# mutiann/few-shot-transformer-tts

Measured on AMD Instinct MI355X. Metric: padded mel-frames/sec, full training step (fwd+loss+bwd+allreduce+Adam), higher is better.
Workload: dtype bf16; 1 GPU; LJSpeech-shaped (BASELINE configs[1]) packed batch per GPU: B=14 S=114 T=582, default hparams (83.5M params), dropout on, single speaker/language; global_batch=14, seq_len=582, parallelism=dp1

## Files before the change

few-shot-transformer-tts_amd/csrc/engine.hip:

```cpp
#include <algorithm>
#include <cmath>
#include <cstdarg>
#include <cstdlib>
#include "engine.h"
#include "attention.h"
#include "enc_fused.h"
#include "drop_sites.h"

thread_local char g_b2s_err[512] = "";
int b2s_fail(const char* file, int line, const char* fmt, ...) {
    char msg[400];
    va_list ap; va_start(ap, fmt); vsnprintf(msg, sizeof(msg), fmt, ap); va_end(ap);
    const char* base = strrchr(file, '/');
    snprintf(g_b2s_err, sizeof(g_b2s_err), "%s:%d: %s", base ? base + 1 : file, line, msg);
    return 1;
}

int b2s_model::id(const std::string& n) const {
    auto it = index.find(n);
    return it == index.end() ? -1 : it->second;
}

namespace {

// ... 1457 lines not shown
            B2S_TRY(ro_cast(dt, memory, c->memT, Mk * D, st));
            if (c->kvcat)
                B2S_TRY(linear(m, st, c->memT, D, m->kv_cat, (int)Mk, cf.n_decoder_layer * 2 * D, D, c->kvcat, 0, cf.n_decoder_layer * 2 * D,
                               GemmEpilogue()));
            return 0;
        };
        if (!memory_ready) B2S_TRY(need_memory());
        if (c->ragged) {
            B2S_TRY(ro_set_rowoff(hoff.data(), B + 1, c->rowoff, st));
            B2S_TRY(ro_rows_gather(dt, targets, c->tgtT, roff, B, T, NM, st));
        } else B2S_TRY(ro_cast(dt, targets, c->tgtT, M * NM, st));
        GemmEpilogue e0; e0.bias = m->P("decoder.prenet.dense0.bias"); e0.relu = 1; e0.drop = make_drop(pd, seed, drop_op(DS_DEC_PRENET0, 0));
        B2S_TRY(linear(m, st, c->tgtT, NM, m->W("decoder.prenet.dense0.weight"), (int)Mr, HP, NM, c->a1, 0, HP, e0));
        GemmEpilogue e1; e1.bias = m->P("decoder.prenet.dense1.bias"); e1.relu = 1; e1.drop = make_drop(pd, seed, drop_op(DS_DEC_PRENET1, 0));
        B2S_TRY(linear(m, st, c->a1, HP, m->W("decoder.prenet.dense1.weight"), (int)Mr, HP, HP, c->a2, 0, HP, e1));
        B2S_TRY(linear(m, st, c->a2, HP, m->W("decoder.prenet.dense_final.weight"), (int)Mr, D, HP, sc.a3, 1, D, GemmEpilogue()));
        B2S_TRY(ro_shift_pe_fwd(sc.a3, target_lengths, m->pe_dec, m->P(p + "pe_scale"), xs[0], B, T, D,
                                make_drop(pt, seed, drop_op(DS_DEC_EMBED, 0)), st, roff, (int)Mr));
        const bool guided = cf.guided_attention_weight > 0.f;
        constexpr bool no_qskip = false;
        const int* qskip = (no_qskip || !padded_unobserved) ? nullptr : target_lengths;
        if (guided) {
            hipLaunchKernelGGL(k_ga_scale, dim3(1), dim3(64), 0, st, input_lengths, target_lengths, B, S, T,
                               cf.guided_attention_weight / (float)(cf.n_decoder_layer * H), c->ga_small);
            if (c->ragged) B2S_HIP(hipMemsetAsync(c->ga_rows, 0, (size_t)cf.n_decoder_layer * B * H * T * sizeof(float), st));
        }
        for (int l = 0; l < cf.n_decoder_layer; ++l) {
            AttnSave& s = c->self_attn[l]; AttnSave& x = c->cross_attn[l]; FfnSave& f = c->ffn[l];
            float* x0 = xs[3 * l]; float* x1 = xs[3 * l + 1]; float* x2 = xs[3 * l + 2]; float* x3 = xs[3 * l + 3];
            const std::string lna = p + "attn_layer_norms." + std::to_string(l);
            B2S_TRY(ro_layernorm_fwd(dt, x0, m->P(lna + ".weight"), m->P(lna + ".bias"), s.h, D, nullptr, 0, s.mean, s.rstd, (int)Mr, D,
                                     1e-6f, nullptr, 1, st));
            B2S_TRY(linear(m, st, s.h, D, m->W(nm(p, "self_attentions", l, "qkv_transform.weight")), (int)Mr, 3 * D, D, s.qkv, 0, 3 * D,
                           GemmEpilogue()));
            s.op_attn = drop_op(DS_DEC_SELF_ATTN, l); s.op_res = drop_op(DS_DEC_SELF_RES, l);
            const char* q = (const char*)s.qkv;
            B2S_TRY(attn_core_fwd(dt, st, q, 3 * D, q + (size_t)D * esz, 3 * D, q + (size_t)2 * D * esz, 3 * D, s.ctx, D, B, H, T, T, dh,
                                  2, nullptr, nullptr, 0, 0, make_drop(pt, seed, s.op_attn), sc.S, s.P, s.Pd, s.lse, nullptr, qskip, roff, roff));
            s.mask_mode = 2; s.qskip = qskip; s.qoff = s.koff = roff;
            GemmEpilogue ea; ea.drop = make_drop(pt, seed, s.op_res); ea.residual = x0; ea.ldr = D;
            B2S_TRY(linear(m, st, s.ctx, D, m->W(nm(p, "self_attentions", l, "output_transform.weight")), (int)Mr, D, D, x1, 1, D, ea));
            const std::string lnx = p + "encdec_layer_norms." + std::to_string(l);
            B2S_TRY(ro_layernorm_fwd(dt, x1, m->P(lnx + ".weight"), m->P(lnx + ".bias"), x.h, D, nullptr, 0, x.mean, x.rstd, (int)Mr, D,
                                     1e-6f, nullptr, 1, st));
            B2S_TRY(linear(m, st, x.h, D, m->W(nm(p, "encdec_attentions", l, "q_transform.weight")), (int)Mr, D, D, x.qkv, 0, D, GemmEpilogue()));
            B2S_TRY(need_memory());
            if (!c->kvcat)
                B2S_TRY(linear(m, st, c->memT, D, m->W(nm(p, "encdec_attentions", l, "kv_transform.weight")), (int)Mk, 2 * D, D, x.kv, 0, 2 * D,
                               GemmEpilogue()));
            x.op_attn = drop_op(DS_DEC_CROSS_ATTN, l); x.op_res = drop_op(DS_DEC_CROSS_RES, l);
            const char* kv = (const char*)x.kv;
            GuidedArgs ga;
            if (guided) {
                ga.rows = c->ga_rows + (long)l * B * H * T; ga.qlen = target_lengths;
                ga.inv2s2 = 1.f / (2.f * cf.guided_attention_sigma * cf.guided_attention_sigma);
            }
            B2S_TRY(attn_core_fwd(dt, st, x.qkv, D, kv, x.ldkv, kv + (size_t)D * esz, x.ldkv, x.ctx, D, B, H, T, S, dh, 1, input_lengths,
                                  nullptr, 0, 0, make_drop(pt, seed, x.op_attn), sc.S, x.P, x.Pd, x.lse, guided ? &ga : nullptr, qskip, roff, nullptr));
            x.mask_mode = 1; x.qskip = qskip; x.qoff = roff;
            GemmEpilogue ex; ex.drop = make_drop(pt, seed, x.op_res); ex.residual = x1; ex.ldr = D;
            B2S_TRY(linear(m, st, x.ctx, D, m->W(nm(p, "encdec_attentions", l, "output_transform.weight")), (int)Mr, D, D, x2, 1, D, ex));
            const std::string lnf = p + "ffn_layer_norms." + std::to_string(l);
            B2S_TRY(ro_layernorm_fwd(dt, x2, m->P(lnf + ".weight"), m->P(lnf + ".bias"), f.h, D, nullptr, 0, f.mean, f.rstd, (int)Mr, D,
                                     1e-6f, nullptr, 1, st));
            f.op_hid = drop_op(DS_DEC_FFN_HID, l); f.op_res = drop_op(DS_DEC_FFN_RES, l);
            GemmEpilogue f1; f1.relu = 1; f1.drop = make_drop(pt, seed, f.op_hid);
            B2S_TRY(linear(m, st, f.h, D, m->W(nm(p, "ffn_layers", l, "input_layer.weight")), (int)Mr, 4 * D, D, f.f, 0, 4 * D, f1));
            GemmEpilogue f2; f2.drop = make_drop(pt, seed, f.op_res); f2.residual = x2; f2.ldr = D;
            B2S_TRY(linear(m, st, f.f, 4 * D, m->W(nm(p, "ffn_layers", l, "output_layer.weight")), (int)Mr, D, 4 * D, x3, 1, D, f2));
        }
        B2S_TRY(need_memory());
        B2S_TRY(ro_layernorm_fwd(dt, c->x_final, m->P(p + "output_layer_norm.weight"), m->P(p + "output_layer_norm.bias"), c->outT, D,
                                 nullptr, 0, c->mean_f, c->rstd_f, (int)Mr, D, 1e-6f, c->ragged ? nullptr : target_lengths, T, st));
        GemmEpilogue em;
        if (!c->ragged) { em.row_len = target_lengths; em.rows_per_batch = T; }
        B2S_TRY(linear(m, st, c->outT, D, m->W("decoder.mel_net.weight"), (int)Mr, NM, D, c->ragged ? c->melc : mels_out, 1, NM, em));
        if (c->ragged)
            B2S_TRY(ro_heads_scatter(dt, c->outT, D, m->P("decoder.stop_net.weight"), m->P("decoder.stop_net.bias"), c->melc, mels_out, stop_out, roff, B, T, NM, D, st));
        else
            B2S_TRY(ro_rowdot_fwd(dt, c->outT, D, m->P("decoder.stop_net.weight"), m->P("decoder.stop_net.bias"), stop_out, (int)Mr, D, target_lengths, T, st));
        if (guided) hipLaunchKernelGGL(k_ga_reduce, dim3(1), dim3(1024), 0, st, c->ga_rows, (long)cf.n_decoder_layer * B * H * T, c->ga_small);
        B2S_LAUNCH_CHECK();
        return 0;
    };
    int rc = run();
    if (rc || !ctx_out) { delete c; if (ctx_out) *ctx_out = nullptr; return rc; }
    *ctx_out = c;
    return 0;
}

namespace {
__global__ void k_rowmask_copy(const float* in, float* out, const int* lens, int T, long n) {
    long i = (long)blockIdx.x * blockDim.x + threadIdx.x;
    if (i < n) { int b = (int)(i / T), t = (int)(i - (long)b * T); out[i] = t < lens[b] ? in[i] : 0.f; }
}
}

extern "C" int b2s_decoder_guided_loss(b2s_model* m, b2s_ctx* c, float* out, float* add_to, void* stream) {
    B2S_CHECK(m && c && c->kind == 2 && out, "bad decoder context");
    B2S_CHECK(c->ga_small, "guided_attention_weight is 0: this forward has no guided-attention term");
    hipLaunchKernelGGL(k_ga_fetch, dim3(1), dim3(1), 0, S_(stream), c->ga_small, out, add_to);
    B2S_LAUNCH_CHECK();
    return 0;
}
extern "C" int b2s_decoder_backward(b2s_model* m, b2s_ctx* c, const float* d_mels, const float* d_stop, const float* d_guided,
                                    int flags, float* d_memory_out, void* dmem_done, void* stream) {
    B2S_TRY(check_bound(m));
    const bool want_dmem = !(flags & B2S_DEC_BWD_NO_DMEMORY);
    B2S_CHECK(c && c->kind == 2 && d_mels && (d_memory_out || !want_dmem), "bad decoder context");
    const b2s_config& cf = m->cfg;
    hipStream_t st = S_(stream);
    const int B = c->B, S = c->S, T = c->T, D = cf.decoder_hidden, H = cf.n_attention_head, dh = D / H, dt = m->dtype, esz = m->esz;
    const int NM = cf.num_mels, HP = cf.prenet_hidden;
    const long Mp = (long)B * T, Mk = (long)B * S;
    const long M = c->ragged ? c->Mr : Mp;
    const int* roff = c->ragged ? c->rowoff : nullptr;
    const float pt = c->train ? cf.transformer_dropout_rate : 0.f, pd = c->train ? cf.decoder_dropout_rate : 0.f;
    Arena a; a.base = c->ws; a.cap = c->ws_bytes;
    b2s_ctx tmp; tmp.B = B; tmp.S = S; tmp.T = T; tmp.train = c->train;
    Scratch sc; std::vector<float*> xs;
    plan_decoder(m, tmp, a, sc, xs);
    const std::string p = "decoder.decoder.";
    const bool guided = c->ga_small != nullptr && d_guided != nullptr;
    if (guided) hipLaunchKernelGGL(k_ga_bscale, dim3(1), dim3(1), 0, st, c->ga_small, d_guided);
    if (c->ragged) B2S_TRY(ro_rows_gather(dt, d_mels, sc.dmelT, roff, B, T, NM, st, d_stop, sc.dstop_m, 1));
    else B2S_TRY(ro_cast(dt, d_mels, sc.dmelT, M * NM, st));
    B2S_TRY(linear_dw(m, st, sc.dmelT, NM, c->outT, D, (int)M, NM, D, m->G("decoder.mel_net.weight")));
    GemmEpilogue eo;
    if (!c->ragged) { eo.row_len = c->tgt_len; eo.rows_per_batch = T; }
    B2S_TRY(linear_dx(m, st, sc.dmelT, NM, m->W("decoder.mel_net.weight"), (int)M, D, NM, sc.doutT, 0, D, eo));
    if (d_stop) {
        if (!c->ragged) hipLaunchKernelGGL(k_rowmask_copy, dim3(cdiv(M, 256)), dim3(256), 0, st, d_stop, sc.dstop_m, c->tgt_len, T, M);
        B2S_TRY(grad_colsum(m, st, dt, c->outT, 0, D, sc.dstop_m, m->G("decoder.stop_net.weight"), 1, (int)M, D));
        B2S_TRY(grad_colsum(m, st, 0, sc.dstop_m, 1, 1, nullptr, m->G("decoder.stop_net.bias"), 1, (int)M, 1));
    }
    DropCfg nd;
    if (cf.n_decoder_layer > 0) nd = make_drop(pt, c->seed, c->ffn[cf.n_decoder_layer - 1].op_res);
    B2S_TRY(ln_bwd_exit(m, st, sc, sc.doutT, 0, D, c->x_final, p + "output_layer_norm", c->mean_f, c->rstd_f, 0, M, D, c->ragged ? nullptr : c->tgt_len, T,
                        cf.n_decoder_layer > 0 ? &nd : nullptr));
    B2S_TRY(end_stage(m, st, 1, false));
#ifdef B2S_LAB
    static const int tail_layers = getenv("B2S_LAB_DW_TAIL_LAYERS") ? atoi(getenv("B2S_LAB_DW_TAIL_LAYERS")) : 1;
    static const int tail_cap = getenv("B2S_LAB_DW_TAIL_CAP") ? atoi(getenv("B2S_LAB_DW_TAIL_CAP")) : 200;
#else
    constexpr int tail_layers = 1;
    constexpr int tail_cap = 200;
#endif
    m->dw_hold_from = -1; m->dw_tail_cap = 0;
    struct TailPolicyReset { b2s_model* m; ~TailPolicyReset() { m->dw_hold_from = -1; m->dw_tail_cap = 0; m->dw_flush_capped = false; } } tail_policy_reset{m};
    if ((flags & B2S_DEC_BWD_FLUSH_TAIL) && m->dw_group && tail_layers > 0 && tail_cap > 0 && dt == 1) {
        m->dw_hold_from = 2 + std::max(0, cf.n_decoder_layer - tail_layers);
        m->dw_tail_cap = tail_cap;
    }
    bool first_mem = true, dmem_finished = false;
    m->side_ev = nullptr;
    struct SideReset { b2s_model* m; ~SideReset() { m->side_ev = nullptr; } } side_reset{m};
    const bool side = m->side && m->side != st && sc.dkvcat && sc.dctx_x && dt == 1 && b2s_flash_supported(dh);
    if (side && m->side_evs.empty()) {
        m->side_evs.resize(16);
        for (auto& e : m->side_evs) B2S_HIP(hipEventCreateWithFlags(&e, hipEventDisableTiming));
    }
    auto finish_dmem = [&]() -> int {
        if (dmem_finished) return 0;
        dmem_finished = true;
        if (m->side_ev) { B2S_HIP(hipStreamWaitEvent(st, m->side_ev, 0)); m->side_ev = nullptr; }
        if (want_dmem && sc.dkvcat && cf.n_decoder_layer > 0) {
            const int Kc = cf.n_decoder_layer * 2 * D;
            GemmArgs g;
            g.A.p = sc.dkvcat; g.A.ld = Kc; g.A.R = (int)Mk; g.A.C = Kc;
            g.B.p = m->kv_cat; g.B.ld = D; g.B.R = Kc; g.B.C = D;
            g.M = (int)Mk; g.N = D; g.K = Kc; g.C = d_memory_out; g.c_fp32 = 1; g.ldc = D;
            if (m->dw_group) {
                B2S_HIP(hipMemsetAsync(d_memory_out, 0, (size_t)Mk * D * 4, st));
                g.epi.accumulate = 1; g.splitk = 4;
                m->set_ws(g, st);
            }
            B2S_TRY(b2s_gemm_launch(g, dt, false, true, st));
        } else if (first_mem && want_dmem) B2S_HIP(hipMemsetAsync(d_memory_out, 0, (size_t)Mk * D * 4, st));
        if (dmem_done) B2S_HIP(hipEventRecord((hipEvent_t)dmem_done, st));
        return 0;
    };
    for (int l = cf.n_decoder_layer - 1; l >= 0; --l) {
        const std::string lnf = p + "ffn_layer_norms." + std::to_string(l), lnx = p + "encdec_layer_norms." + std::to_string(l),
                          lna = p + "attn_layer_norms." + std::to_string(l);
        nd = make_drop(pt, c->seed, c->cross_attn[l].op_res);
        B2S_TRY(ffn_bwd(m, st, c->ffn[l], sc, M, D, pt, c->seed, nm(p, "ffn_layers", l, "input_layer.weight"),
                        nm(p, "ffn_layers", l, "output_layer.weight"), lnf, &nd));
        {
            const AttnSave& x = c->cross_attn[l];
            const std::string wq = nm(p, "encdec_attentions", l, "q_transform.weight"), wkv = nm(p, "encdec_attentions", l, "kv_transform.weight"),
                              wo = nm(p, "encdec_attentions", l, "output_transform.weight");
            DropCfg dres = make_drop(pt, c->seed, x.op_res), datt = make_drop(pt, c->seed, x.op_attn);
            const void* dy;
            B2S_TRY(take_dy(m, st, sc, M, D, dres, &dy));
            B2S_TRY(linear_dw(m, st, dy, D, x.ctx, D, (int)M, D, D, m->G(wo)));
            void* const dctx = side ? sc.dctx_x : sc.dctx;
            float* const dsum = side ? sc.dsum_x : sc.dP;
            if (side && m->side_ev) B2S_HIP(hipStreamWaitEvent(st, m->side_ev, 0));
            B2S_TRY(linear_dx(m, st, dy, D, m->W(wo), (int)M, D, D, dctx, 0, D, GemmEpilogue()));
            sc.dqkv = Scratch::rot(sc.r_dqkv, sc.i_dqkv);
            B2S_TRY(guard_write(m, sc.dqkv, st));
            int lddkv = 2 * D;
            if (sc.dkvcat) { sc.dkv = (char*)sc.dkvcat + (size_t)l * 2 * D * esz; lddkv = cf.n_decoder_layer * 2 * D; }
            else { sc.dkv = Scratch::rot(sc.r_dkv, sc.i_dkv); B2S_TRY(guard_write(m, sc.dkv, st)); }
            const char* kv = (const char*)x.kv; char* dkv = (char*)sc.dkv;
            GuidedArgs ga;
            if (guided) {
                ga.rows = c->ga_rows + (long)l * B * H * T; ga.qlen = c->tgt_len; ga.scale = c->ga_small + 2;
                ga.inv2s2 = 1.f / (2.f * cf.guided_attention_sigma * cf.guided_attention_sigma);
            }
            B2S_TRY(attn_core_bwd(dt, st, dctx, D, x.qkv, D, kv, x.ldkv, kv + (size_t)D * esz, x.ldkv, x.P, x.Pd, sc.dqkv, D, dkv, lddkv,
                                  dkv + (size_t)D * esz, lddkv, B, H, T, S, dh, datt, dsum, sc.dS, x.lse, x.ctx, x.mask_mode, c->in_len,
                                  guided ? &ga : nullptr, x.qskip, x.qoff, x.koff, side ? m->side : nullptr, side ? m->next_event() : nullptr));
            if (side) {
                hipEvent_t e = m->side_evs[m->side_next++ % m->side_evs.size()];
                B2S_HIP(hipEventRecord(e, m->side));
                m->side_ev = e;
            }
            B2S_TRY(linear_dw(m, st, sc.dqkv, D, x.h, D, (int)M, D, D, m->G(wq)));
            B2S_TRY(linear_dx(m, st, sc.dqkv, D, m->W(wq), (int)M, D, D, sc.dh, 0, D, GemmEpilogue()));
            B2S_TRY(linear_dw(m, st, sc.dkv, lddkv, c->memT, D, (int)Mk, 2 * D, D, m->G(wkv)));
            if (want_dmem && !sc.dkvcat) {
                GemmEpilogue em; em.accumulate = first_mem ? 0 : 1;
                B2S_TRY(linear_dx(m, st, sc.dkv, 2 * D, m->W(wkv), (int)Mk, D, 2 * D, d_memory_out, 1, D, em));
                first_mem = false;
            }
            if (l == 0) B2S_TRY(finish_dmem());
            nd = make_drop(pt, c->seed, c->self_attn[l].op_res);
            B2S_TRY(ln_bwd_exit(m, st, sc, sc.dh, 0, D, x.x_in, lnx, x.mean, x.rstd, 1, M, D, nullptr, 1, &nd));
        }
        if (l > 0) nd = make_drop(pt, c->seed, c->ffn[l - 1].op_res);
        B2S_TRY(self_attn_bwd(m, st, c->self_attn[l], sc, M, D, B, H, T, pt, c->seed, nm(p, "self_attentions", l, "qkv_transform.weight"),
                              nm(p, "self_attentions", l, "output_transform.weight"), lna, nullptr, l > 0 ? &nd : nullptr));
        B2S_TRY(end_stage(m, st, 2 + (cf.n_decoder_layer - 1 - l), false));
    }
    B2S_TRY(finish_dmem());
    B2S_TRY(ro_shift_pe_bwd(dt, sc.dx, c->tgt_len, m->pe_dec, sc.da3, m->G(p + "pe_scale"), B, T, D, make_drop(pt, c->seed, drop_op(DS_DEC_EMBED, 0)), st, m->dx_bf16,
                            roff, (int)M));
    DropCfg d1 = make_drop(pd, c->seed, drop_op(DS_DEC_PRENET0, 0)), d2 = make_drop(pd, c->seed, drop_op(DS_DEC_PRENET1, 0));
    B2S_TRY(linear_dw(m, st, sc.da3, D, c->a2, HP, (int)M, D, HP, m->G("decoder.prenet.dense_final.weight")));
    GemmEpilogue e2; e2.relu_aux = c->a2; e2.ld_aux = HP; e2.aux_scale = d2.scale;
    B2S_TRY(linear_dx(m, st, sc.da3, D, m->W("decoder.prenet.dense_final.weight"), (int)M, HP, D, sc.dz2, 0, HP, e2));
    B2S_TRY(grad_colsum(m, st, dt, sc.dz2, 0, HP, nullptr, m->G("decoder.prenet.dense1.bias"), 1, (int)M, HP));
    B2S_TRY(linear_dw(m, st, sc.dz2, HP, c->a1, HP, (int)M, HP, HP, m->G("decoder.prenet.dense1.weight")));
    GemmEpilogue e1; e1.relu_aux = c->a1; e1.ld_aux = HP; e1.aux_scale = d1.scale;
    B2S_TRY(linear_dx(m, st, sc.dz2, HP, m->W("decoder.prenet.dense1.weight"), (int)M, HP, HP, sc.dz1, 0, HP, e1));
    B2S_TRY(grad_colsum(m, st, dt, sc.dz1, 0, HP, nullptr, m->G("decoder.prenet.dense0.bias"), 1, (int)M, HP));
    B2S_TRY(linear_dw(m, st, sc.dz1, HP, c->tgtT, NM, (int)M, HP, NM, m->G("decoder.prenet.dense0.weight")));
    B2S_LAUNCH_CHECK();
    if (flags & B2S_DEC_BWD_FLUSH_TAIL) {
#ifdef B2S_LAB
        static const bool lab_early_mark = getenv("B2S_LAB_EARLY_MARK") != nullptr;
        if (lab_early_mark && m->aux) {
            if (!m->grads_mark_ev) B2S_HIP(hipEventCreateWithFlags(&m->grads_mark_ev, hipEventDisableTiming));
            B2S_HIP(hipEventRecord(m->grads_mark_ev, m->aux));
            m->lab_early_marked = true;
        }
#endif
        m->dw_flush_capped = m->dw_hold_from >= 0;
        m->dw_hold_from = -1;
        const int rc = end_stage(m, st, 2 + cf.n_decoder_layer, false, true);
        m->dw_flush_capped = false;
        return rc;
    }
    m->dw_hold_from = -1;
    B2S_TRY(end_stage(m, st, 2 + cf.n_decoder_layer, !(flags & B2S_DEC_BWD_DEFER_JOIN)));
    return 0;
}

extern "C" int b2s_decoder_alignment(b2s_model* m, b2s_ctx* c, int which, int layer, float* out, void* stream) {
    B2S_CHECK(m && c && c->kind == 2 && out, "bad decoder context");
    B2S_CHECK(layer >= 0 && layer < m->cfg.n_decoder_layer && (which == 0 || which == 1), "bad alignment selector");
    const AttnSave& s = which ? c->cross_attn[layer] : c->self_attn[layer];
    if (s.lse) {
        const int D = m->cfg.decoder_hidden, H = m->cfg.n_attention_head, dh = D / H, esz = m->esz;
        AttnArgs a;
        if (which) a = flash_args(s.qkv, D, s.kv, s.ldkv, nullptr, 0, c->B, H, s.Lq, s.Lk, dh, 1, c->in_len, DropCfg{0, 0, 1.f}, s.lse);
        else a = flash_args(s.qkv, 3 * D, (const char*)s.qkv + (size_t)D * esz, 3 * D, nullptr, 0, c->B, H, s.Lq, s.Lk, dh, 2, nullptr, DropCfg{0, 0, 1.f}, s.lse);
        a.qskip = s.qskip; a.qoff = s.qoff; a.koff = s.koff;
        return b2s_flash_align(m->dtype, a, dh, out, S_(stream));
    }
    return ro_align_transpose(m->dtype, s.P, out, c->B * m->cfg.n_attention_head, s.Lq, s.Lk, s.ldp, S_(stream));
}

extern "C" size_t b2s_postnet_ws_bytes(const b2s_model* m, int B, int T) {
    if (!m || B <= 0 || T <= 0) return 0;
    b2s_ctx c; c.B = B; c.T = T;
    Arena a; PostScratch ps;
    plan_postnet(m, c, a, ps);
    return a.off + 4096;
}

extern "C" int b2s_postnet_forward(b2s_model* m, const float* inputs, const int32_t* lengths, const float* add, int B, int T,
                                   int train, uint64_t seed, void* ws, size_t ws_bytes, float* out, void* stream,
                                   b2s_ctx** ctx_out) {
    B2S_TRY(check_bound(m));
    const b2s_config& cf = m->cfg;
    B2S_CHECK(inputs && lengths && out && ws && B > 0 && T > 0, "bad argument");
    B2S_CHECK(!train || (long)B * T > 1, "Expected more than 1 value per channel when training, got B=%d T=%d (BatchNorm batch statistics)", B, T);
    hipStream_t st = S_(stream);
    b2s_ctx* c = new b2s_ctx();
    c->kind = 3; c->B = B; c->T = T; c->train = train; c->seed = seed; c->tgt_len = lengths;
    c->ws = (char*)ws; c->ws_bytes = ws_bytes;
    Arena a; a.base = (char*)ws; a.cap = ws_bytes;
    PostScratch ps;
    plan_postnet(m, *c, a, ps);
    if (a.overflow || a.off > ws_bytes) { delete c; return b2s_fail(__FILE__, __LINE__, "postnet workspace too small: need %zu bytes, got %zu", a.off, ws_bytes); }
    const long M = (long)B * T;
    const int n = cf.n_postnet_layer, dt = m->dtype;
    const float pd = train ? cf.decoder_dropout_rate : 0.f;
    const bool fused_stats = train != 0;
    auto run = [&]() -> int {
        B2S_TRY(ro_cast(dt, inputs, c->u[0], M * cf.num_mels, st));
        if (fused_stats) B2S_HIP(hipMemsetAsync(ps.stat, 0, sizeof(float) * (size_t)n * ps.stat_stride, st));
        for (int i = 0; i < n; ++i) {
            const int cin = i == 0 ? cf.num_mels : cf.postnet_hidden, cout = i == n - 1 ? cf.num_mels : cf.postnet_hidden;
            const std::string q = "postnet.batchnorm_layers." + std::to_string(i) + ".";
            float* sums = ps.stat + (size_t)i * ps.stat_stride;
            GemmArgs g;
            g.A.p = c->u[i]; g.A.ld = cin; g.A.R = (int)M; g.A.C = 5 * cin; g.A.g_cin = cin; g.A.g_T = T; g.A.g_len = lengths;
            g.B.p = m->conv_wf[i]; g.B.ld = 5 * cin; g.B.R = cout; g.B.C = 5 * cin;
            g.M = (int)M; g.N = cout; g.K = 5 * cin; g.C = c->y[i]; g.c_fp32 = 1; g.ldc = cout;
            if (fused_stats) g.epi.colstat = sums;
            B2S_TRY(b2s_gemm_launch(g, dt, false, false, st));
            DropCfg d = make_drop(pd, seed, drop_op(DS_POST_CONV, i));
            const bool last = i == n - 1;
            if (fused_stats) {
                B2S_TRY(ro_bn_apply_train(dt, c->y[i], sums, c->bn_mean[i], c->bn_rstd[i], 1e-5f, m->P(q + "running_mean"), m->P(q + "running_var"),
                                          (long*)m->data[m->id(q + "num_batches_tracked")], 0.1f, m->P(q + "weight"), m->P(q + "bias"), last ? 0 : 1,
                                          last ? nullptr : c->u[i + 1], last ? out : nullptr, last ? add : nullptr, (int)M, cout, d, st));
                continue;
            }
            B2S_TRY(ro_bn_eval_stats(m->P(q + "running_mean"), m->P(q + "running_var"), c->bn_mean[i], c->bn_rstd[i], 1e-5f, cout, st));
            if (!last)
                B2S_TRY(ro_bn_apply(dt, c->y[i], c->bn_mean[i], c->bn_rstd[i], m->P(q + "weight"), m->P(q + "bias"), 1, c->u[i + 1],
                                    nullptr, nullptr, (int)M, cout, d, st));
            else
                B2S_TRY(ro_bn_apply(dt, c->y[i], c->bn_mean[i], c->bn_rstd[i], m->P(q + "weight"), m->P(q + "bias"), 0, nullptr, out,
                                    add, (int)M, cout, d, st));
        }
        return 0;
    };
    int rc = run();
    if (rc || !ctx_out) { delete c; if (ctx_out) *ctx_out = nullptr; return rc; }
    *ctx_out = c;
    return 0;
}

extern "C" int b2s_postnet_backward(b2s_model* m, b2s_ctx* c, const float* d_out, float* d_inputs_out, int flags, void* stream) {
    B2S_TRY(check_bound(m));
    B2S_CHECK(c && c->kind == 3 && d_out && d_inputs_out, "bad postnet context");
    B2S_CHECK(c->train, "postnet backward requires a train-mode forward (batch statistics)");
    const b2s_config& cf = m->cfg;
    hipStream_t st = S_(stream);
    const int B = c->B, T = c->T, n = cf.n_postnet_layer, dt = m->dtype;
    const long M = (long)B * T;
    const float pd = cf.decoder_dropout_rate;
    Arena a; a.base = c->ws; a.cap = c->ws_bytes;
    b2s_ctx tmp; tmp.B = B; tmp.T = T;
    PostScratch ps;
    plan_postnet(m, tmp, a, ps);
    std::vector<GemmArgs> dws, segs;
    for (int i = n - 1; i >= 0; --i) {
        const int cin = i == 0 ? cf.num_mels : cf.postnet_hidden, cout = i == n - 1 ? cf.num_mels : cf.postnet_hidden;
        const std::string q = "postnet.batchnorm_layers." + std::to_string(i) + ".";
        DropCfg d = make_drop(pd, c->seed, drop_op(DS_POST_CONV, i));
        const void* dout = i == n - 1 ? (const void*)d_out : ps.du[i + 1];
        void* dy = ps.dy[i];
        B2S_TRY(ro_bn_bwd(dt, dout, i == n - 1 ? 1 : 0, c->y[i], c->bn_mean[i], c->bn_rstd[i], m->P(q + "weight"), m->P(q + "bias"),
                          i < n - 1 ? 1 : 0, m->G(q + "weight"), m->G(q + "bias"), dy, (int)M, cout, d, st));
        if (dt == 1 && cin % 8 == 0 && cout % 8 == 0) {
            GemmArgs g;
            g.A.p = dy; g.A.ld = cout; g.B.p = c->u[i]; g.B.ld = cin;
            g.M = cout; g.N = cin; g.K = (int)M;
            g.C = m->G("postnet.conv_layers." + std::to_string(i) + ".weight"); g.c_fp32 = 1; g.ldc = 5 * cin;
            g.epi.accumulate = 1;
            segs.push_back(g);
        } else {
            GemmArgs g;
            g.A.p = dy; g.A.ld = cout; g.A.R = (int)M; g.A.C = cout;
            g.B.p = c->u[i]; g.B.ld = cin; g.B.R = (int)M; g.B.C = 5 * cin; g.B.g_cin = cin; g.B.g_T = T; g.B.g_len = c->tgt_len;
            g.M = cout; g.N = 5 * cin; g.K = (int)M;
            g.C = m->G("postnet.conv_layers." + std::to_string(i) + ".weight"); g.c_fp32 = 1; g.ldc = 5 * cin;
            g.epi.conv_dw_cin = cin; g.epi.accumulate = 1; g.splitk = pick_splitk(cout, 5 * cin, (int)M, dt);
            if (m->aux) dws.push_back(g);
            else { m->set_ws(g, st); B2S_TRY(b2s_gemm_launch(g, dt, true, true, st)); }
        }
        {
            GemmArgs g;
            g.A.p = dy; g.A.ld = cout; g.A.R = (int)M; g.A.C = 5 * cout; g.A.g_cin = cout; g.A.g_T = T; g.A.g_len = nullptr;
            g.B.p = m->conv_wb[i]; g.B.ld = 5 * cout; g.B.R = cin; g.B.C = 5 * cout;
            g.M = (int)M; g.N = cin; g.K = 5 * cout;
            g.epi.row_len = c->tgt_len; g.epi.rows_per_batch = T;
            if (i == 0) { g.C = d_inputs_out; g.c_fp32 = 1; } else { g.C = ps.du[i]; g.c_fp32 = 0; }
            g.ldc = cin;
            B2S_TRY(b2s_gemm_launch(g, dt, false, false, st));
        }
    }
    auto launch_segs = [&](hipStream_t s) -> int {
        for (size_t i = 0; i < segs.size(); i += B2S_MAX_GROUP)
            B2S_TRY(b2s_gemm_conv_dw_launch(segs.data() + i, (int)std::min<size_t>(B2S_MAX_GROUP, segs.size() - i), c->tgt_len, B, T, s));
        return 0;
// ... 229 lines not shown
```

few-shot-transformer-tts_amd/csrc/gemm.h:

```cpp
#pragma once
#include "b2s_common.h"

struct GemmOperand {
    const void* p = nullptr;
    long bs_o = 0, bs_i = 0;
    int ld = 0;
    int R = 0, C = 0;
    int g_cin = 0, g_T = 0;
    const int* g_len = nullptr;
};

struct GemmEpilogue {
    float alpha = 1.f;
    const float* bias = nullptr;
    int relu = 0;
    const void* relu_aux = nullptr;
    int ld_aux = 0;
    float aux_scale = 1.f;
    DropCfg drop = {0, 0, 1.f};
    const int* drop_salt = nullptr;
    const float* residual = nullptr;
    int ldr = 0;
    const int* row_len = nullptr;
    int rows_per_batch = 1;
    int conv_dw_cin = 0;
    int accumulate = 0;
    float* colstat = nullptr;
    void *kv_k = nullptr, *kv_v = nullptr;
    const int* kv_t = nullptr;
    int kv_maxT = 0, kv_D = 0, kv_dh = 0;
};

struct GemmArgs {
    GemmOperand A, B;
    int M = 0, N = 0, K = 0;
    int batch = 1, batch_inner = 1;
    int splitk = 1;
    void* C = nullptr;
    int c_fp32 = 0;
    int ldc = 0;
    long cs_o = 0, cs_i = 0;
    GemmEpilogue epi;
    float* ws = nullptr;
    size_t ws_floats = 0;
};

int b2s_gemm_launch(const GemmArgs& g, int dtype, bool ta, bool tb, hipStream_t stream);
int b2s_gemm_glds_launch(const GemmArgs& g, bool ta, bool tb, hipStream_t stream);
int b2s_gemm_skinny_launch(const GemmArgs& g, int dtype, hipStream_t stream);
long b2s_gemm_glds256_tiles(const GemmArgs& g);
int b2s_gemm_glds256_launch(const GemmArgs& g, bool ta, bool tb, const bf16_t* zero, hipStream_t stream);
int b2s_splitk_reduce_launch(const float* ws, float* dst, int M, int N, int ldc, int splitk, int conv_dw_cin, hipStream_t stream);
#define B2S_MAX_GROUP 8
struct b2s_gemm_group { int n; int order; int tile0[B2S_MAX_GROUP + 1]; GemmArgs p[B2S_MAX_GROUP];
                        const int* seg_len; int seg_n, seg_T; };
int b2s_gemm_glds256_grouped_launch(const GemmArgs* probs, int n, const bf16_t* zero, hipStream_t stream);
int b2s_gemm_glds256_conv_dw_launch(const GemmArgs* probs, int n, const int* len, int B, int T, const bf16_t* zero, hipStream_t stream);
int b2s_gemm_conv_dw_launch(const GemmArgs* probs, int n, const int* len, int B, int T, hipStream_t stream);
const bf16_t* b2s_gemm_zero_page();
int b2s_gemm_grouped_launch(const GemmArgs* probs, int n, hipStream_t stream);
```

few-shot-transformer-tts_amd/csrc/gemm_glds256.hip:

```cpp
#include <algorithm>
#include <vector>
#include <cstdlib>
#include <mutex>
#include <atomic>
#include "gemm.h"
#include "gemm_epi.h"

#ifndef B2S_DMA_AUX
#define B2S_DMA_AUX 0
#endif

#ifndef B2S_GROUP_M
#define B2S_GROUP_M 4
#endif
#ifndef B2S_NPROD
#define B2S_NPROD 4
#endif

namespace t256 {

constexpr int NPROD = B2S_NPROD, GROUP_M = B2S_GROUP_M;
constexpr int nprod_of(int gather, int mw = 4) { return gather == 1 ? 0 : NPROD * mw / 4; }
constexpr int nthreads_of(int gather, int mw = 4) { return 64 * (2 * mw + nprod_of(gather, mw)); }
template <int N> __device__ __forceinline__ void wait_vm() { asm volatile("s_waitcnt vmcnt(%0)" ::"n"(N) : "memory"); }
// ... 611 lines not shown
    DropCfg dcfg = g.epi.drop;
    if (dcfg.thresh && g.epi.drop_salt) dcfg.key ^= b2s_hash32((uint32_t)(*g.epi.drop_salt) * 2246822519u + 3266489917u);
    const unsigned stg = lds_base + (unsigned)(PST_STG + wave * 1024);
    f32x4_t acc[4][NB];
    bf16x8_t fa0[4], fb0[4], fa1[4], fb1[4];
    __builtin_amdgcn_s_barrier();
    int slot = 0;
    int v = (int)blockIdx.x;
    for (int t = 0; v != PST_END; ++t) {
        int m0, n0; tile_at(v, m0, n0);
#pragma unroll
        for (int a = 0; a < 4; ++a)
#pragma unroll
            for (int b = 0; b < NB; ++b) acc[a][b] = (f32x4_t){0.f, 0.f, 0.f, 0.f};
        B2S_READ8(fa0, fb0, slot, 0)
        asm volatile("s_waitcnt lgkmcnt(0)" ::: "memory");
        __builtin_amdgcn_sched_barrier(0);
        for (int kt = 0; kt < nk; ++kt) {
            const int nslot = slot + 1 == NSTAGE ? 0 : slot + 1;
            B2S_READ8(fa1, fb1, slot, 1)
            __builtin_amdgcn_sched_barrier(0);
            B2S_MMA16(fa0, fb0)
            __builtin_amdgcn_sched_barrier(0);
            asm volatile("s_waitcnt lgkmcnt(0)" ::: "memory");
            __builtin_amdgcn_s_barrier();
            B2S_READ8(fa0, fb0, nslot, 0)
            __builtin_amdgcn_sched_barrier(0);
            B2S_MMA16(fa1, fb1)
            __builtin_amdgcn_sched_barrier(0);
            asm volatile("s_waitcnt lgkmcnt(0)" ::: "memory");
            __builtin_amdgcn_sched_barrier(0);
            slot = nslot;
        }
        __builtin_amdgcn_sched_barrier(0);
        v = queued(t + 1);
        if (mode == 0) epi_small<NB, 0>(ef, dcfg, acc, stg, m0 + wrow, n0 + wcol, lane);
        else if (mode == 1 && !dcfg.thresh) epi_small<NB, 1>(ef, dcfg, acc, stg, m0 + wrow, n0 + wcol, lane);
        else if (mode == 1) epi_small<NB, 3>(ef, dcfg, acc, stg, m0 + wrow, n0 + wcol, lane);
        else epi_small<NB, 2>(ef, dcfg, acc, stg, m0 + wrow, n0 + wcol, lane);
        __builtin_amdgcn_sched_barrier(0);
    }
#undef B2S_READ8
#undef B2S_MMA16
}

inline int persist_mode(const GemmArgs& g) {
    const GemmEpilogue& e = g.epi;
    if (g.c_fp32 || e.residual || e.bias || e.row_len || e.alpha != 1.f || e.kv_k || e.accumulate || e.conv_dw_cin || e.colstat) return -1;
    if ((g.ldc & 7) || (reinterpret_cast<uintptr_t>(g.C) & 15) || g.cs_o || g.cs_i) return -1;
    if (!e.relu && !e.relu_aux && !e.drop.thresh) return 0;
    if (e.relu && !e.relu_aux) return 1;
    if (e.relu_aux && !e.relu && !e.drop.thresh && (e.ld_aux & 7) == 0 && (reinterpret_cast<uintptr_t>(e.relu_aux) & 15) == 0) return 2;
    return -1;
}
#ifdef B2S_LAB
static const int g_persist = getenv("B2S_LAB_GEMM_PERSIST") ? atoi(getenv("B2S_LAB_GEMM_PERSIST")) : 1;
static const int g_persist_min = getenv("B2S_LAB_GEMM_PERSIST_MIN") ? atoi(getenv("B2S_LAB_GEMM_PERSIST_MIN")) : 1;
#else
constexpr int g_persist = 1;
constexpr int g_persist_min = 1;
#endif
int* persist_ticket_set() {
    constexpr int MAXDEV = 16;
    static int* pool[MAXDEV] = {};
    static std::once_flag once[MAXDEV];
    int dev = 0;
    if (hipGetDevice(&dev) != hipSuccess || dev < 0 || dev >= MAXDEV) { (void)hipGetLastError(); return nullptr; }
    std::call_once(once[dev], [dev] {
        void* p = nullptr;
        if (hipMalloc(&p, 1024 * 64) == hipSuccess && hipMemset(p, 0, 1024 * 64) == hipSuccess) pool[dev] = (int*)p;
        else (void)hipGetLastError();
    });
    static std::atomic<unsigned> next{0};
    return pool[dev] ? pool[dev] + (next.fetch_add(1, std::memory_order_relaxed) & 1023u) * 16 : nullptr;
}
template <bool TB, int NB>
int launch256_persist(const GemmArgs& g, int mode, hipStream_t stream) {
    constexpr size_t smem = PST_LDS;
    static std::once_flag attr_once;
    static hipError_t attr_err = hipSuccess;
    std::call_once(attr_once, [] {
        attr_err = hipFuncSetAttribute(reinterpret_cast<const void*>(gemm_glds256_persist_kernel<TB, NB>), hipFuncAttributeMaxDynamicSharedMemorySize, (int)smem);
    });
    B2S_HIP(attr_err);
    const int tiles_m = cdiv(g.M, BM), tiles_n = g.N / (NB * 32);
    int* tickets = (g_persist == 2 || tiles_m * tiles_n <= 256) ? nullptr : persist_ticket_set();
    const int grid = std::min(256, tiles_m * tiles_n);
    hipLaunchKernelGGL((gemm_glds256_persist_kernel<TB, NB>), dim3(grid), dim3(nthreads_of(0, 4)), smem, stream, g, tiles_m, tiles_n, mode, tickets);
    B2S_LAUNCH_CHECK();
    return 0;
}
template <bool TA, bool TB, int GATHER, int NB>
int try_persist(const GemmArgs& g, hipStream_t stream) {
    if (TA || GATHER != 0 || !g_persist) return -1;
    const long tiles = (long)cdiv(g.M, BM) * cdiv(g.N, NB * 32);
    if (tiles < g_persist_min || (tiles < 256 && (tiles & 7)) || tiles >= (1 << 24) || g.batch != 1 || g.splitk != 1 || g.K < 6 * BK || g.K % BK != 0 || g.N % (NB * 32) != 0) return -1;
    if ((long)g.A.R * g.A.ld >= (1L << 30) || (long)g.B.R * g.B.ld >= (1L << 30) || g.A.g_cin || g.B.g_cin) return -1;
    if (TB && !(g.B.C >= 8 && (g.B.C & 7) == 0)) return -1;
    const int mode = persist_mode(g);
    if (mode < 0) return -1;
    return launch256_persist<TB, NB>(g, mode, stream);
}

template <bool TA, bool TB, int GATHER, int NB, int MW = 4>
int launch256_nb(const GemmArgs& g_in, const bf16_t* zero, hipStream_t stream) {
    GemmArgs g = g_in;
    if (g.splitk > 1) {
        const int nk_all = cdiv(g.K, BK), per = cdiv(nk_all, g.splitk);
        g.splitk = cdiv(nk_all, per);
    }
    constexpr size_t smem = (size_t)NSTAGE * (MW * 64 * BK * 2 + B_BYTES);
    static std::once_flag attr_once;
    static hipError_t attr_err = hipSuccess;
    std::call_once(attr_once, [] {
        attr_err = hipFuncSetAttribute(reinterpret_cast<const void*>(gemm_glds256_kernel<TA, TB, GATHER, NB, MW>),
                                       hipFuncAttributeMaxDynamicSharedMemorySize, (int)smem);
    });
    B2S_HIP(attr_err);
    const int tiles_m = cdiv(g.M, MW * 64), tiles_n = cdiv(g.N, NB * 32);
    dim3 grid(tiles_m * tiles_n * g.batch * g.splitk);
    float* ws = nullptr;
    if (g.splitk > 1 && g.batch == 1 && g.c_fp32 && g.epi.accumulate && (g.N & 3) == 0 && (g.ldc & 3) == 0 &&
        g.ws && (size_t)g.splitk * g.M * g.N <= g.ws_floats)
        ws = g.ws;
    hipLaunchKernelGGL((gemm_glds256_kernel<TA, TB, GATHER, NB, MW>), grid, dim3(nthreads_of(GATHER, MW)), smem, stream, g, zero, ws, tiles_m, tiles_n);
    B2S_LAUNCH_CHECK();
    if (ws) B2S_TRY(b2s_splitk_reduce_launch(ws, (float*)g.C, g.M, g.N, g.ldc, g.splitk, g.epi.conv_dw_cin, stream));
    return 0;
}

std::atomic<int> g_tile_policy{0};
inline int pick_nb(const GemmArgs& g, bool allow64 = false) {
    static const int env_force = getenv("B2S_GEMM256_NB") ? atoi(getenv("B2S_GEMM256_NB")) : 0;
    const int force = env_force ? env_force : g_tile_policy.load(std::memory_order_relaxed);
    if (force == 3 || force == 4) return force;
    const long per = (long)cdiv(g.M, BM) * g.batch * std::max(1, g.splitk);
    const long r128 = (per * cdiv(g.N, 128) + 255) / 256 * 128, r96 = (per * cdiv(g.N, 96) + 255) / 256 * 101;
    if (allow64) {
        const long r64 = (per * cdiv(g.N, 64) + 255) / 256 * 72;
        if (r64 < std::min(r96, r128)) return 2;
    }
    return r96 < r128 ? 3 : 4;
}
template <bool TA, bool TB, int GATHER>
int launch256_t(const GemmArgs& g, const bf16_t* zero, hipStream_t stream) {
    if (!TA && GATHER == 0) {
#ifdef B2S_LAB
        static const int small_tiles = getenv("B2S_LAB_SMALL_TILES") ? atoi(getenv("B2S_LAB_SMALL_TILES")) : 128;
#else
        constexpr int small_tiles = 128;
#endif
        const int nb = pick_nb(g);
        const long t256n = (long)cdiv(g.M, BM) * cdiv(g.N, nb * 32) * g.batch * std::max(1, g.splitk);
        if (t256n <= small_tiles && g.M > 128) {
            constexpr bool ta = false;
            return nb == 3 ? launch256_nb<ta, TB, 0, 3, 2>(g, zero, stream)
                           : launch256_nb<ta, TB, 0, 4, 2>(g, zero, stream);
        }
    }
#ifdef B2S_LAB
    static const bool lab_no64 = getenv("B2S_LAB_NO_NB2") != nullptr;
#else
    constexpr bool lab_no64 = false;
#endif
    const int nb = pick_nb(g, GATHER == 2 && !TB && !lab_no64);
    if constexpr (GATHER == 2 && !TB) {
        if (nb == 2) return launch256_nb<TA, TB, GATHER, 2>(g, zero, stream);
    }
    const int rc = nb == 3 ? try_persist<TA, TB, GATHER, 3>(g, stream) : try_persist<TA, TB, GATHER, 4>(g, stream);
    if (rc >= 0) return rc;
    return nb == 3 ? launch256_nb<TA, TB, GATHER, 3>(g, zero, stream)
                   : launch256_nb<TA, TB, GATHER, 4>(g, zero, stream);
}

}

int b2s_gemm_glds256_grouped_launch(const GemmArgs* probs, int n, const bf16_t* zero, hipStream_t stream) {
    B2S_CHECK(n >= 1 && n <= B2S_MAX_GROUP, "grouped GEMM: %d problems (max %d)", n, B2S_MAX_GROUP);
    b2s_gemm_group grp;
    grp.n = n;
    grp.order = 1;
    int order[B2S_MAX_GROUP];
    auto makespan = [&](bool deep_first) {
        for (int i = 0; i < n; ++i) order[i] = i;
        std::stable_sort(order, order + n, [&](int a, int b) { return deep_first ? probs[a].K > probs[b].K : probs[a].K < probs[b].K; });
        std::vector<long> cu(256, 0);
        auto cmp = [](long a, long b) { return a > b; };
        long end = 0;
        for (int k = 0; k < n; ++k) {
            const GemmArgs& g = probs[order[k]];
            const int t = cdiv(g.M, t256::BM) * cdiv(g.N, 128);
            for (int j = 0; j < t; ++j) {
                std::pop_heap(cu.begin(), cu.end(), cmp);
                cu.back() += g.K + 1024;
                end = std::max(end, cu.back());
                std::push_heap(cu.begin(), cu.end(), cmp);
            }
        }
        return end;
    };
    const long deep = makespan(true), shallow = makespan(false);
    if (deep <= shallow) makespan(true);
    int tiles = 0;
    for (int k = 0; k < n; ++k) {
        const GemmArgs& g = probs[order[k]];
        B2S_CHECK(g.batch == 1 && g.c_fp32 && g.A.g_cin == 0 && g.B.g_cin == 0, "grouped GEMM: problem %d is not a plain fp32 dW", order[k]);
        grp.p[k] = g; grp.p[k].splitk = 1;
        grp.tile0[k] = tiles;
        tiles += cdiv(g.M, t256::BM) * cdiv(g.N, 128);
    }
    grp.tile0[n] = tiles;
    grp.seg_len = nullptr; grp.seg_n = 0; grp.seg_T = 0;
    constexpr size_t smem = (size_t)t256::NSTAGE * t256::STAGE_BYTES;
    static std::once_flag attr_once;
    static hipError_t attr_err = hipSuccess;
    std::call_once(attr_once, [] {
        attr_err = hipFuncSetAttribute(reinterpret_cast<const void*>(t256::gemm_glds256_grouped_kernel<4>),
                                       hipFuncAttributeMaxDynamicSharedMemorySize, (int)smem);
    });
    B2S_HIP(attr_err);
    hipLaunchKernelGGL((t256::gemm_glds256_grouped_kernel<4>), dim3(tiles), dim3(t256::nthreads_of(false)), smem, stream, grp, zero);
    B2S_LAUNCH_CHECK();
    return 0;
}

int b2s_gemm_glds256_conv_dw_launch(const GemmArgs* probs, int n, const int* len, int B, int T, const bf16_t* zero, hipStream_t stream) {
    B2S_CHECK(n >= 1 && n <= B2S_MAX_GROUP && B > 0 && T > 0 && (long)B * T < (1L << 30), "conv dW: %d layers (max %d), B = %d, T = %d", n, B2S_MAX_GROUP, B, T);
    b2s_gemm_group grp;
    grp.n = n; grp.order = 1;
    grp.seg_len = len; grp.seg_n = B; grp.seg_T = T;
    int tiles = 0;
    for (int k = 0; k < n; ++k) {
        GemmArgs g = probs[k];
        B2S_CHECK(g.batch == 1 && g.c_fp32 && g.A.p && g.B.p && g.C && g.A.g_cin == 0 && g.B.g_cin == 0, "conv dW: layer %d is not a plain fp32 dW", k);
        B2S_CHECK(g.M > 0 && g.N > 0 && g.M % 8 == 0 && g.N % 8 == 0 && g.A.ld % 8 == 0 && g.B.ld % 8 == 0 && g.A.ld >= g.M && g.B.ld >= g.N && g.ldc >= 5 * g.N,
                  "conv dW: layer %d: cout = %d, cin = %d and the leading dimensions (%d, %d) must be multiples of 8, ldc = %d >= 5 cin", k, g.M, g.N,
                  g.A.ld, g.B.ld, g.ldc);
        B2S_CHECK(((uintptr_t)g.A.p % 16 == 0) && ((uintptr_t)g.B.p % 16 == 0), "conv dW: operands must be 16-byte aligned");
        B2S_CHECK(!g.epi.bias && !g.epi.relu && !g.epi.relu_aux && !g.epi.residual && !g.epi.drop.thresh && !g.epi.row_len && !g.epi.colstat && !g.epi.kv_k,
                  "conv dW: linear epilogue only");
        g.A.R = g.B.R = g.K = B * T; g.A.C = g.M; g.B.C = g.N;
        g.splitk = 1; g.ws = nullptr; g.ws_floats = 0; g.cs_o = g.cs_i = 0; g.A.bs_o = g.A.bs_i = g.B.bs_o = g.B.bs_i = 0;
        g.epi.conv_dw_cin = g.N;
        grp.p[k] = g;
        grp.tile0[k] = tiles;
        tiles += cdiv(g.M, t256::BM) * 5 * cdiv(g.N, 128);
    }
    grp.tile0[n] = tiles;
    constexpr size_t smem = (size_t)t256::NSTAGE * t256::STAGE_BYTES;
    static std::once_flag attr_once;
    static hipError_t attr_err = hipSuccess;
    std::call_once(attr_once, [] {
        attr_err = hipFuncSetAttribute(reinterpret_cast<const void*>(t256::gemm_glds256_grouped_kernel<4, true>),
                                       hipFuncAttributeMaxDynamicSharedMemorySize, (int)smem);
    });
    B2S_HIP(attr_err);
    hipLaunchKernelGGL((t256::gemm_glds256_grouped_kernel<4, true>), dim3(tiles), dim3(t256::nthreads_of(false)), smem, stream, grp, zero);
    B2S_LAUNCH_CHECK();
    return 0;
}

extern "C" int b2s_gemm_set_tile_policy(int policy) {
    if (policy != 0 && policy != 3 && policy != 4) return b2s_fail(__FILE__, __LINE__, "tile policy must be 0 (auto), 3 (256x96) or 4 (256x128), got %d", policy);
    t256::g_tile_policy.store(policy, std::memory_order_relaxed);
    return 0;
}

long b2s_gemm_glds256_tiles(const GemmArgs& g) { return (long)cdiv(g.M, t256::BM) * cdiv(g.N, 128) * g.batch * std::max(1, g.splitk); }

int b2s_gemm_glds256_launch(const GemmArgs& g, bool ta, bool tb, const bf16_t* zero, hipStream_t stream) {
    const bool gather = g.A.g_cin > 0 || g.B.g_cin > 0;
    if (gather) {
        if (!ta && !tb) {
            const bool aligned = g.A.g_cin > 0 && g.B.g_cin == 0 && g.A.g_cin % t256::BK == 0 && g.K % t256::BK == 0 && g.splitk == 1 &&
                                 (long)g.A.R * g.A.ld < (1L << 29) && (long)g.B.R * g.B.ld < (1L << 30) && g.A.g_T > 0;
            if (aligned) return t256::launch256_t<false, false, 2>(g, zero, stream);
            return t256::launch256_t<false, false, 1>(g, zero, stream);
        }
        if (ta && tb) return t256::launch256_t<true, true, 1>(g, zero, stream);
        return b2s_fail(__FILE__, __LINE__, "conv gather is supported for the NT and TN forms only");
    }
    if (!ta && !tb) return t256::launch256_t<false, false, 0>(g, zero, stream);
    if (!ta && tb) return t256::launch256_t<false, true, 0>(g, zero, stream);
    if (ta && !tb) return t256::launch256_t<true, false, 0>(g, zero, stream);
    return t256::launch256_t<true, true, 0>(g, zero, stream);
}
```

Baseline: 1.264 million mel-frames/s.

## Split decoder memory-gradient GEMM into pieces overlapped on side stream

Replaces the single end-of-loop memory-gradient GEMM over the concatenated dkv buffer with two pieces. The piece covering layers 1..L-1 launches once layer 1's dkv is ready, and the layer-0 piece accumulates later. Both run on the side stream when available, so they overlap with main-stream decoder backward work, and a join event at the tail syncs back. This drops the memset and split-k path and adds event bookkeeping, at the risk of contention with main-stream kernels.

Result: no change. 1.273 million mel-frames/s, median of 6 (+0.7%).

```diff
diff --git a/few-shot-transformer-tts_amd/csrc/engine.hip b/few-shot-transformer-tts_amd/csrc/engine.hip
--- a/few-shot-transformer-tts_amd/csrc/engine.hip
+++ b/few-shot-transformer-tts_amd/csrc/engine.hip
@@ -1633,7 +1633,7 @@
         m->dw_hold_from = 2 + std::max(0, cf.n_decoder_layer - tail_layers);
         m->dw_tail_cap = tail_cap;
     }
-    bool first_mem = true, dmem_finished = false;
+    bool first_mem = true;
     m->side_ev = nullptr;
     struct SideReset { b2s_model* m; ~SideReset() { m->side_ev = nullptr; } } side_reset{m};
     const bool side = m->side && m->side != st && sc.dkvcat && sc.dctx_x && dt == 1 && b2s_flash_supported(dh);
@@ -1641,24 +1641,28 @@
         m->side_evs.resize(16);
         for (auto& e : m->side_evs) B2S_HIP(hipEventCreateWithFlags(&e, hipEventDisableTiming));
     }
-    auto finish_dmem = [&]() -> int {
-        if (dmem_finished) return 0;
-        dmem_finished = true;
-        if (m->side_ev) { B2S_HIP(hipStreamWaitEvent(st, m->side_ev, 0)); m->side_ev = nullptr; }
-        if (want_dmem && sc.dkvcat && cf.n_decoder_layer > 0) {
-            const int Kc = cf.n_decoder_layer * 2 * D;
-            GemmArgs g;
-            g.A.p = sc.dkvcat; g.A.ld = Kc; g.A.R = (int)Mk; g.A.C = Kc;
-            g.B.p = m->kv_cat; g.B.ld = D; g.B.R = Kc; g.B.C = D;
-            g.M = (int)Mk; g.N = D; g.K = Kc; g.C = d_memory_out; g.c_fp32 = 1; g.ldc = D;
-            if (m->dw_group) {
-                B2S_HIP(hipMemsetAsync(d_memory_out, 0, (size_t)Mk * D * 4, st));
-                g.epi.accumulate = 1; g.splitk = 4;
-                m->set_ws(g, st);
-            }
-            B2S_TRY(b2s_gemm_launch(g, dt, false, true, st));
-        } else if (first_mem && want_dmem) B2S_HIP(hipMemsetAsync(d_memory_out, 0, (size_t)Mk * D * 4, st));
-        if (dmem_done) B2S_HIP(hipEventRecord((hipEvent_t)dmem_done, st));
+    const hipStream_t sk = side ? m->side : st;
+    auto dmem_piece = [&](int l0, int l1, int accumulate) -> int {
+        const int Kc = cf.n_decoder_layer * 2 * D, Kp = (l1 - l0) * 2 * D;
+        GemmArgs g;
+        g.A.p = (const char*)sc.dkvcat + (size_t)l0 * 2 * D * esz; g.A.ld = Kc; g.A.R = (int)Mk; g.A.C = Kp;
+        g.B.p = (const char*)m->kv_cat + (size_t)l0 * 2 * D * D * esz; g.B.ld = D; g.B.R = Kp; g.B.C = D;
+        g.M = (int)Mk; g.N = D; g.K = Kp; g.C = d_memory_out; g.c_fp32 = 1; g.ldc = D;
+        g.epi.accumulate = accumulate;
+#ifdef B2S_LAB
+        static const int lab_rows_a = getenv("B2S_LAB_DMEM_ROWS_A") ? atoi(getenv("B2S_LAB_DMEM_ROWS_A")) : 0;
+        static const int lab_rows_b = getenv("B2S_LAB_DMEM_ROWS_B") ? atoi(getenv("B2S_LAB_DMEM_ROWS_B")) : 0;
+        g.tile_rows = l0 > 0 ? lab_rows_a : lab_rows_b;
+#endif
+        return b2s_gemm_launch(g, dt, false, true, sk);
+    };
+    const bool pieces = want_dmem && sc.dkvcat != nullptr;
+    struct SideJoin { hipStream_t st; hipEvent_t ev = nullptr; ~SideJoin() { if (ev) (void)hipStreamWaitEvent(st, ev, 0); } } side_tail{st};
+    auto side_record = [&](bool dkv) -> int {
+        hipEvent_t e = m->side_evs[m->side_next++ % m->side_evs.size()];
+        B2S_HIP(hipEventRecord(e, m->side));
+        side_tail.ev = e;
+        if (dkv) m->side_ev = e;
         return 0;
     };
     for (int l = cf.n_decoder_layer - 1; l >= 0; --l) {
@@ -1693,10 +1697,11 @@
             B2S_TRY(attn_core_bwd(dt, st, dctx, D, x.qkv, D, kv, x.ldkv, kv + (size_t)D * esz, x.ldkv, x.P, x.Pd, sc.dqkv, D, dkv, lddkv,
                                   dkv + (size_t)D * esz, lddkv, B, H, T, S, dh, datt, dsum, sc.dS, x.lse, x.ctx, x.mask_mode, c->in_len,
                                   guided ? &ga : nullptr, x.qskip, x.qoff, x.koff, side ? m->side : nullptr, side ? m->next_event() : nullptr));
-            if (side) {
-                hipEvent_t e = m->side_evs[m->side_next++ % m->side_evs.size()];
-                B2S_HIP(hipEventRecord(e, m->side));
-                m->side_ev = e;
+            if (pieces && l == 0) B2S_TRY(dmem_piece(0, 1, cf.n_decoder_layer > 1 ? 1 : 0));
+            if (side) B2S_TRY(side_record(true));
+            if (pieces && l == 1) {
+                B2S_TRY(dmem_piece(1, cf.n_decoder_layer, 0));
+                if (side) B2S_TRY(side_record(false));
             }
             B2S_TRY(linear_dw(m, st, sc.dqkv, D, x.h, D, (int)M, D, D, m->G(wq)));
             B2S_TRY(linear_dx(m, st, sc.dqkv, D, m->W(wq), (int)M, D, D, sc.dh, 0, D, GemmEpilogue()));
@@ -1706,7 +1711,7 @@
                 B2S_TRY(linear_dx(m, st, sc.dkv, 2 * D, m->W(wkv), (int)Mk, D, 2 * D, d_memory_out, 1, D, em));
                 first_mem = false;
             }
-            if (l == 0) B2S_TRY(finish_dmem());
+            if (l == 0 && dmem_done) B2S_HIP(hipEventRecord((hipEvent_t)dmem_done, sk));
             nd = make_drop(pt, c->seed, c->self_attn[l].op_res);
             B2S_TRY(ln_bwd_exit(m, st, sc, sc.dh, 0, D, x.x_in, lnx, x.mean, x.rstd, 1, M, D, nullptr, 1, &nd));
         }
@@ -1715,7 +1720,10 @@
                               nm(p, "self_attentions", l, "output_transform.weight"), lna, nullptr, l > 0 ? &nd : nullptr));
         B2S_TRY(end_stage(m, st, 2 + (cf.n_decoder_layer - 1 - l), false));
     }
-    B2S_TRY(finish_dmem());
+    if (cf.n_decoder_layer == 0) {
+        if (want_dmem) B2S_HIP(hipMemsetAsync(d_memory_out, 0, (size_t)Mk * D * 4, st));
+        if (dmem_done) B2S_HIP(hipEventRecord((hipEvent_t)dmem_done, st));
+    }
     B2S_TRY(ro_shift_pe_bwd(dt, sc.dx, c->tgt_len, m->pe_dec, sc.da3, m->G(p + "pe_scale"), B, T, D, make_drop(pt, c->seed, drop_op(DS_DEC_EMBED, 0)), st, m->dx_bf16,
                             roff, (int)M));
     DropCfg d1 = make_drop(pd, c->seed, drop_op(DS_DEC_PRENET0, 0)), d2 = make_drop(pd, c->seed, drop_op(DS_DEC_PRENET1, 0));
@@ -1729,6 +1737,7 @@
     B2S_TRY(grad_colsum(m, st, dt, sc.dz1, 0, HP, nullptr, m->G("decoder.prenet.dense0.bias"), 1, (int)M, HP));
     B2S_TRY(linear_dw(m, st, sc.dz1, HP, c->tgtT, NM, (int)M, HP, NM, m->G("decoder.prenet.dense0.weight")));
     B2S_LAUNCH_CHECK();
+    if (side_tail.ev) { B2S_HIP(hipStreamWaitEvent(st, side_tail.ev, 0)); side_tail.ev = nullptr; m->side_ev = nullptr; }
     if (flags & B2S_DEC_BWD_FLUSH_TAIL) {
 #ifdef B2S_LAB
         static const bool lab_early_mark = getenv("B2S_LAB_EARLY_MARK") != nullptr;
diff --git a/few-shot-transformer-tts_amd/csrc/gemm.h b/few-shot-transformer-tts_amd/csrc/gemm.h
--- a/few-shot-transformer-tts_amd/csrc/gemm.h
+++ b/few-shot-transformer-tts_amd/csrc/gemm.h
@@ -36,6 +36,7 @@
     int M = 0, N = 0, K = 0;
     int batch = 1, batch_inner = 1;
     int splitk = 1;
+    int tile_rows = 0;
     void* C = nullptr;
     int c_fp32 = 0;
     int ldc = 0;
diff --git a/few-shot-transformer-tts_amd/csrc/gemm_glds256.hip b/few-shot-transformer-tts_amd/csrc/gemm_glds256.hip
--- a/few-shot-transformer-tts_amd/csrc/gemm_glds256.hip
+++ b/few-shot-transformer-tts_amd/csrc/gemm_glds256.hip
@@ -787,7 +787,7 @@
 #endif
         const int nb = pick_nb(g);
         const long t256n = (long)cdiv(g.M, BM) * cdiv(g.N, nb * 32) * g.batch * std::max(1, g.splitk);
-        if (t256n <= small_tiles && g.M > 128) {
+        if (t256n <= small_tiles && g.M > 128 && g.tile_rows != 256) {
             constexpr bool ta = false;
             return nb == 3 ? launch256_nb<ta, TB, 0, 3, 2>(g, zero, stream)
                            : launch256_nb<ta, TB, 0, 4, 2>(g, zero, stream);
```
